# jqsl2012/RL_CTR_Prediction

Measured on NVIDIA B200. Metric: train samples/sec, higher is better.
Workload: dtype f32

## Files before the change

rl_ctr_prediction_b200/csrc/optim.cu:

```cuda
#include <cub/device/device_radix_sort.cuh>

#include <cstdlib>

#include "common.cuh"

namespace rlctr {

constexpr int LONG_RUN = 32;

struct TableView {
    float* data;
    int64_t n_rows;
    int rs, lin_col, emb_col, dim;
    int pitch;
    int used;
};
static inline TableView view_of(const rlctr_table* t) {
    int used = t->emb_col + t->dim;
    if (t->lin_col + 1 > used) used = t->lin_col + 1;
    if (used < 1) used = 1;
    return TableView{t->data, t->n_rows, t->row_stride, t->lin_col, t->emb_col, t->dim,
                     t->row_pitch > 0 ? t->row_pitch : t->row_stride, used};
}
struct AdamView {
    float* m;
    float* v;
    int32_t* stamp;
    int stamp_col;
    const float2* sched;
    const int32_t* step;
    AdamHyper h;
    const float* stage;
    int stage_pitch;
};
static inline int stage_pitch_of(const TableView& t) { return t.rs == 1 ? 4 : 3 * ((t.used + 3) & ~3); }
static inline AdamView view_of(const rlctr_adam* a, const TableView& t) {
    return AdamView{a->exp_avg, a->exp_avg_sq, a->stamp_col >= 0 ? nullptr : a->stamp, a->stamp_col >= 0 ? a->stamp_col : -1,
                    reinterpret_cast<const float2*>(a->sched), a->step,
                    adam_hyper(a->beta1, a->beta2, a->eps, a->weight_decay), a->stage, stage_pitch_of(t)};
}
__device__ __forceinline__ bool is_lazy(const AdamView& a) { return a.stamp != nullptr || a.stamp_col >= 0; }
__device__ __forceinline__ int load_stamp(const TableView& t, const AdamView& a, int64_t id) {
    return a.stamp_col >= 0 ? __float_as_int(t.data[id * t.pitch + a.stamp_col]) : a.stamp[id];
}
__device__ __forceinline__ void embed_stamp(float4& p, int col0, const AdamView& a, int value) {
    if (a.stamp_col >= 0 && (a.stamp_col & ~3) == col0) f4set(p, a.stamp_col & 3, __int_as_float(value));
}
struct GroupCols {
    int n;
    const float* dz[RLCTR_GROUP_MAX];
    const float* extra[RLCTR_GROUP_MAX];
    int emb_col[RLCTR_GROUP_MAX], dim[RLCTR_GROUP_MAX];
    const uint32_t* slot_of;
    int sums_pitch;
    signed char member[32];
    signed char role[32];
    int dz_used;
};
struct GradView {
    GroupCols grp;
    const float* staged;
    const float* dlogit;
    const float* sums;
    const float* extra;
    int fields;
    int flags;
    int world;
    uint32_t n_per_rank;
    const float* p_staged[RLCTR_MAX_WORLD];
    const float* p_dlogit[RLCTR_MAX_WORLD];
    const float* p_sums[RLCTR_MAX_WORLD];
    const float* p_extra[RLCTR_MAX_WORLD];
};
struct GradSrc {
    const float* staged;
    const float* dlogit;
    const float* sums;
    const float* extra;
    uint32_t slot;
};
__device__ __forceinline__ GradSrc grad_src(const GradView& g, uint32_t slot) {
    if (g.world <= 1) return GradSrc{g.staged, g.dlogit, g.sums, g.extra, slot};
    const uint32_t src = slot / g.n_per_rank;
    return GradSrc{g.p_staged[src], g.p_dlogit[src], g.p_sums[src], g.p_extra[src], slot - src * g.n_per_rank};
}
static inline GradView grad_view_of(const rlctr_rowgrad* grad) {
    GradView g{};
    g.staged = grad->staged; g.dlogit = grad->dlogit; g.sums = grad->sums; g.extra = grad->extra;
    g.fields = grad->fields; g.flags = grad->flags;
    g.world = grad->world; g.n_per_rank = grad->n_per_rank;
    if (grad->world > 1) {
        for (int r = 0; r < grad->world && r < RLCTR_MAX_WORLD; ++r) {
            g.p_staged[r] = grad->peer_staged[r]; g.p_dlogit[r] = grad->peer_dlogit[r];
            g.p_sums[r] = grad->peer_sums[r]; g.p_extra[r] = grad->peer_extra[r];
        }
        g.staged = grad->peer_staged[0]; g.dlogit = grad->peer_dlogit[0]; g.sums = grad->peer_sums[0]; g.extra = grad->peer_extra[0];
    }
    return g;
}

__global__ void __launch_bounds__(256)
sort_prep_kernel(const int64_t* __restrict__ ids, int64_t n, int64_t n_rows, uint32_t* __restrict__ keys,
                 uint32_t* __restrict__ vals) {
    for (int64_t i = (int64_t)blockIdx.x * blockDim.x + threadIdx.x; i < n; i += (int64_t)gridDim.x * blockDim.x) {
        const int64_t id = __ldg(ids + i);
        keys[i] = ((uint64_t)id < (uint64_t)n_rows) ? (uint32_t)id : (uint32_t)n_rows;
        vals[i] = (uint32_t)i;
    }
}

__global__ void __launch_bounds__(256)
sort_prep_sharded_kernel(const uint32_t* __restrict__ ids_all, int64_t n_all, int64_t n_rows_global, int shift, uint32_t mask,
                         uint32_t rank, uint32_t n_local, uint32_t* __restrict__ keys, uint32_t* __restrict__ vals) {
    for (int64_t i = (int64_t)blockIdx.x * blockDim.x + threadIdx.x; i < n_all; i += (int64_t)gridDim.x * blockDim.x) {
        const uint32_t id = __ldg(ids_all + i);
        const bool mine = (uint64_t)id < (uint64_t)n_rows_global && (id & mask) == rank;
        keys[i] = mine ? (id >> shift) : n_local;
        vals[i] = (uint32_t)i;
    }
}

struct GradRaw {
    float4 r;
    float4 S;
    float dz;
    float ex[4];
    bool fm, has_ex, any;
};
__device__ __forceinline__ GradRaw rowgrad_load(const GradView& g, uint32_t gslot, int col0, const TableView& t) {
    const GradSrc q = grad_src(g, gslot);
    const uint32_t slot = q.slot;
    GradRaw w;
    w.r = f4zero(); w.S = f4zero(); w.dz = 0.f; w.fm = false; w.has_ex = false; w.any = false;
#pragma unroll
    for (int k = 0; k < 4; ++k) w.ex[k] = 0.f;
    if (q.staged) w.r = ldg4(q.staged + (int64_t)slot * t.rs + col0);
    if (g.flags & RLCTR_STAGED_PARTNER) {
        w.dz = __ldg(q.dlogit + slot / (uint32_t)g.fields);
        return w;
    }
    if (q.dlogit || q.extra) {
        w.any = true;
        const uint32_t b = slot / (uint32_t)g.fields;
        const uint32_t f = slot - b * (uint32_t)g.fields;
        w.fm = q.sums && q.dlogit;
        if (w.fm && (g.flags & RLCTR_DZ_IN_SUMS)) w.dz = __ldg(q.sums + (int64_t)b * t.rs + (t.rs - 1));
        else if (q.dlogit) w.dz = __ldg(q.dlogit + b);
        if (w.fm) w.S = ldg4(q.sums + (int64_t)b * t.rs + col0);
        if (q.extra) {
            w.has_ex = true;
            const float* ex = q.extra + ((int64_t)b * g.fields + f) * t.dim;
#pragma unroll
            for (int k = 0; k < 4; ++k) {
                const int col = col0 + k;
                if (col >= t.emb_col && col < t.emb_col + t.dim) w.ex[k] = __ldg(ex + col - t.emb_col);
            }
        }
    }
    return w;
}
__device__ __forceinline__ float4 rowgrad_combine(const GradView& g, const GradRaw& w, int col0, const float4& p, const TableView& t) {
    float4 r = w.r;
    if (g.flags & RLCTR_STAGED_PARTNER) return make_float4(w.dz * r.x, w.dz * r.y, w.dz * r.z, w.dz * r.w);
    if (w.any) {
#pragma unroll
        for (int k = 0; k < 4; ++k) {
            const int col = col0 + k;
            float add = 0.f;
            if (col == t.lin_col) {
                add = w.dz;
            } else if (col >= t.emb_col && col < t.emb_col + t.dim) {
                if (w.fm) add = __fmul_rn(w.dz, f4get(w.S, k) - f4get(p, k));
                if (w.has_ex) add = __fadd_rn(add, w.ex[k]);
            }
            f4set(r, k, __fadd_rn(f4get(r, k), add));
        }
    }
    return r;
}
struct GroupLane {
    int mem[4], role[4];
};
__device__ __forceinline__ GroupLane group_lane(const GradView& g, int col0) {
    GroupLane gl;
#pragma unroll
    for (int k = 0; k < 4; ++k) {
        const int col = col0 + k;
        gl.mem[k] = col < 32 ? (int)g.grp.member[col] : -1;
        gl.role[k] = col < 32 ? (int)g.grp.role[col] : 0;
    }
    return gl;
}
__device__ __forceinline__ float group_col_grad(int role, float dz, float S, float p, bool has_ex, float ex) {
    float add = 0.f;
    if (role == 1) {
        add = dz;
    } else if (role != 0) {
        if (role == 2) add = __fmul_rn(dz, S - p);
        if (has_ex) add = __fadd_rn(add, ex);
    }
    return __fadd_rn(0.f, add);
}
__device__ __forceinline__ float4 rowgrad_group(const GradView& g, const GroupLane& gl, uint32_t slot, int col0, const float4& p,
                                                const TableView& t) {
    const uint32_t erow = slot;
    if (g.grp.slot_of) slot = __ldg(g.grp.slot_of + slot);
    const uint32_t b = slot / (uint32_t)g.fields;
    const float* srow = g.sums + (int64_t)b * g.grp.sums_pitch;
    const float4 S = ldg4(srow + col0);
    float4 r = f4zero();
#pragma unroll
    for (int k = 0; k < 4; ++k) {
        const int m = gl.mem[k];
        if (m < 0) continue;
        const float* dzp = g.grp.dz[m];
        const bool want_dz = gl.role[k] == 1 || gl.role[k] == 2;
        const float dz = !want_dz ? 0.f : dzp ? __ldg(dzp + b) : __ldg(srow + g.grp.sums_pitch - RLCTR_GROUP_MAX + m);
        const float* ex = gl.role[k] >= 2 ? g.grp.extra[m] : nullptr;
        const float exv = ex ? __ldg(ex + (int64_t)erow * g.grp.dim[m] + (col0 + k - g.grp.emb_col[m])) : 0.f;
        f4set(r, k, group_col_grad(gl.role[k], dz, f4get(S, k), f4get(p, k), ex != nullptr, exv));
    }
    return r;
}
template <bool GROUP>
__device__ __forceinline__ float4 rowgrad_any(const GradView& g, const GroupLane& gl, uint32_t slot, int col0, const float4& p,
                                              const TableView& t) {
    if (GROUP) return rowgrad_group(g, gl, slot, col0, p, t);
    return rowgrad_combine(g, rowgrad_load(g, slot, col0, t), col0, p, t);
}
__device__ __forceinline__ float4 rowgrad_chunk(const GradView& g, uint32_t gslot, int col0, const float4& p,
                                                const TableView& t) {
    return rowgrad_combine(g, rowgrad_load(g, gslot, col0, t), col0, p, t);
}

__device__ __forceinline__ void adam_apply4(float4& p, float4& m, float4& v, const float4& g, float2 s,
                                            const AdamHyper& h) {
    const float ib = rcp_approx(s.y);
    adam_elem_fast(p.x, m.x, v.x, g.x, h, s.x, ib);
    adam_elem_fast(p.y, m.y, v.y, g.y, h, s.x, ib);
    adam_elem_fast(p.z, m.z, v.z, g.z, h, s.x, ib);
    adam_elem_fast(p.w, m.w, v.w, g.w, h, s.x, ib);
}

template <int APPLY>
__device__ __forceinline__ void finish_row(int64_t id, int col0, float4 p, const float4& acc, const TableView& t,
                                           const AdamView& a, float* dense_grad, int step, int stamp_in,
                                           const float4* m_pre = nullptr, const float4* v_pre = nullptr) {
    if (APPLY == 1) {
        st4(dense_grad + id * t.rs + col0, acc);
        return;
    }
    const int64_t off = id * t.pitch + col0;
    float4 m = m_pre ? *m_pre : ld4(a.m + off), v = v_pre ? *v_pre : ld4(a.v + off);
    if (is_lazy(a) && !a.stage && stamp_in < step - 1) adam_replay4(p, m, v, stamp_in, step - 1, a.sched, a.h);
    adam_apply4(p, m, v, acc, __ldg(&a.sched[step]), a.h);
    embed_stamp(p, col0, a, step);
    st4(t.data + off, p);
    st4(a.m + off, m);
    st4(a.v + off, v);
}
// ... 981 lines not shown
    float* m[RLCTR_DENSE_MAX];
    float* v[RLCTR_DENSE_MAX];
    int64_t n[RLCTR_DENSE_MAX];
    int first_block[RLCTR_DENSE_MAX + 1];
    int step_index[RLCTR_DENSE_MAX];
    int count;
};
__global__ void __launch_bounds__(256)
dense_adam_multi_kernel(const __grid_constant__ DenseGroup grp, const float2* __restrict__ sched, const int32_t* __restrict__ steps,
                        AdamHyper h) {
    int t = 0;
    while (t + 1 < grp.count && (int)blockIdx.x >= grp.first_block[t + 1]) ++t;
    const float2 sc = __ldg(&sched[__ldg(steps + grp.step_index[t]) + 1]);
    const int nb = grp.first_block[t + 1] - grp.first_block[t];
    float* __restrict__ p = grp.p[t];
    const float* __restrict__ g = grp.g[t];
    float* __restrict__ m = grp.m[t];
    float* __restrict__ v = grp.v[t];
    for (int64_t i = (int64_t)(blockIdx.x - grp.first_block[t]) * blockDim.x + threadIdx.x; i < grp.n[t]; i += (int64_t)nb * blockDim.x) {
        float pp = p[i], mm = m[i], vv = v[i];
        adam_elem(pp, mm, vv, g[i], h, sc.x, sc.y);
        p[i] = pp; m[i] = mm; v[i] = vv;
    }
}

static inline int grid_1d(int64_t threads, int cap_blocks) {
    int64_t blocks = (threads + 255) / 256;
    if (blocks < 1) blocks = 1;
    return (int)(blocks < cap_blocks ? blocks : cap_blocks);
}
static inline int key_bits(int64_t n_rows) {
    int b = 1;
    while (b < 32 && ((int64_t)1 << b) <= n_rows) ++b;
    return b;
}
struct RowsWs {
    int32_t* long_count;
    uint32_t* long_list;
};
static inline size_t rows_ws_bytes(int64_t n) { return 16 + sizeof(uint32_t) * (size_t)(n / LONG_RUN + 1); }

static inline unsigned capped_blocks(int64_t full, int world) {
    if (world <= 1) return (unsigned)full;
    int64_t cap = full / world + full / (4 * world) + 2 * RLCTR_SMS;
    return (unsigned)(cap < full ? cap : full);
}

static inline int rows_grid_env() {
    static int v = -1;
    if (v < 0) { const char* e = getenv("RLCTR_ROWS_GRID"); v = e ? atoi(e) : 1; }
    return v;
}

template <int APPLY>
static int launch_rows(const uint32_t* sorted_ids, const uint32_t* sorted_slots, int64_t n, const rlctr_rowgrad* grad,
                       const rlctr_table* table, const rlctr_adam* opt, float* dense_grad, void* ws, size_t ws_bytes,
                       cudaStream_t st) {
    if (!sorted_ids || !sorted_slots || !grad || !table || !table->data || n < 0) return RLCTR_EINVAL;
    if (APPLY == 0 && (!opt || !opt->exp_avg || !opt->exp_avg_sq || !opt->sched || !opt->step)) return RLCTR_EINVAL;
    if (APPLY == 0 && opt->stamp_col >= (table->row_pitch > 0 ? table->row_pitch : table->row_stride)) return RLCTR_EINVAL;
    if (APPLY == 0 && opt->stamp_col >= 0 && table->row_stride > 32) return RLCTR_EUNSUPPORTED;
    if (APPLY == 1 && !dense_grad) return RLCTR_EINVAL;
    if ((grad->dlogit || grad->extra) && grad->fields <= 0) return RLCTR_EINVAL;
    if (n == 0) return RLCTR_OK;
    TableView t = view_of(table);
    AdamView a = APPLY == 0 ? view_of(opt, t) : AdamView{};
    if (grad->world > RLCTR_MAX_WORLD || (grad->world > 1 && grad->n_per_rank == 0)) return RLCTR_EINVAL;
    GradView g = grad_view_of(grad);
    if ((g.flags & RLCTR_STAGED_PARTNER) && (!g.staged || !g.dlogit || g.fields <= 0)) return RLCTR_EINVAL;
    if ((g.flags & RLCTR_DZ_IN_SUMS) && (t.rs <= t.used || !g.sums)) return RLCTR_EINVAL;
    if (t.rs == 1) {
        if (grad->extra || grad->sums) return RLCTR_EUNSUPPORTED;
        rows_scalar_kernel<APPLY><<<capped_blocks((n + 255) / 256, grad->world), 256, 0, st>>>(sorted_ids, sorted_slots, n, g, t, a,
                                                                                              dense_grad);
        RLCTR_LAUNCH_CHECK();
        return RLCTR_OK;
    }
    if (t.rs % 4 != 0 || t.rs > 128 * WCH) return RLCTR_EUNSUPPORTED;
    if (t.rs > 32) {
        rows_wide_kernel<APPLY><<<(unsigned)((n + 7) / 8), 256, 0, st>>>(sorted_ids, sorted_slots, n, g, t, a, dense_grad);
        RLCTR_LAUNCH_CHECK();
        return RLCTR_OK;
    }
    if (ws_bytes < rows_ws_bytes(n) || !ws) return RLCTR_EWORKSPACE;
    RowsWs w{reinterpret_cast<int32_t*>(ws), reinterpret_cast<uint32_t*>(reinterpret_cast<char*>(ws) + 16)};
    RLCTR_CUDA(cudaMemsetAsync(w.long_count, 0, sizeof(int32_t), st));
    const int lpr = rlctr_lanes_per_row(t.rs);
    unsigned blocks = capped_blocks((n * lpr + 255) / 256, grad->world);
    if (rows_grid_env() > 0 && blocks > (unsigned)(RLCTR_SMS * 5 * rows_grid_env())) blocks = RLCTR_SMS * 5 * rows_grid_env();
#define LAUNCH_ROWS(L)                                                                                              \
    rows_short_kernel<L, APPLY><<<blocks, 256, 0, st>>>(sorted_ids, sorted_slots, n, g, t, a, dense_grad,           \
                                                        w.long_count, w.long_list);                                \
    rows_long_kernel<L, APPLY><<<RLCTR_SMS, 256, 0, st>>>(sorted_ids, sorted_slots, n, g, t, a, dense_grad,         \
                                                          w.long_count, w.long_list)
    if (APPLY == 0 && a.stage && a.stamp == nullptr && lpr <= 4) {
        static int r_env = -1;
        if (r_env < 0) { const char* e = getenv("RLCTR_ROWS_R"); r_env = e ? atoi(e) : 0; }
        if (r_env == 0 && lpr == 4) {
            const int ch = (t.used + 3) >> 2;
            const int64_t tiles = capped_blocks((n + tile::TT - 1) / tile::TT, grad->world);
            const unsigned tb = (unsigned)(tiles < RLCTR_SMS * 3 ? tiles : RLCTR_SMS * 3);
#define LAUNCH_TILE(C)                                                                                                \
            { const size_t sm = 2 * sizeof(tile::Buf<C>);                                                             \
              RLCTR_CUDA(cudaFuncSetAttribute(rows_staged_tile_kernel<C>, cudaFuncAttributeMaxDynamicSharedMemorySize, (int)sm)); \
              rows_staged_tile_kernel<C><<<tb, 256, sm, st>>>(sorted_ids, sorted_slots, n, g, t, a, w.long_count, w.long_list); }
            switch (ch) {
                case 1: LAUNCH_TILE(1); break;
                case 2: LAUNCH_TILE(2); break;
                case 3: LAUNCH_TILE(3); break;
                default: LAUNCH_TILE(4); break;
            }
#undef LAUNCH_TILE
            RLCTR_LAUNCH_CHECK();
            rows_long_kernel<4, 0><<<RLCTR_SMS, 256, 0, st>>>(sorted_ids, sorted_slots, n, g, t, a, dense_grad, w.long_count, w.long_list);
            RLCTR_LAUNCH_CHECK();
            return RLCTR_OK;
        }
        const int R = r_env == 2 ? 2 : 4;
        const int64_t per_block = (256 / lpr) * R;
        int64_t want = (n + per_block - 1) / per_block;
        want = capped_blocks(want, grad->world);
        const int64_t cap = (int64_t)RLCTR_SMS * (R > 2 ? 2 : 3) * 4;
        const unsigned sblocks = (unsigned)(want < cap ? want : cap);
#define LAUNCH_STAGED(L)                                                                                              \
        if (R == 2) rows_staged_kernel<L, 2><<<sblocks, 256, 0, st>>>(sorted_ids, sorted_slots, n, g, t, a, w.long_count, w.long_list); \
        else rows_staged_kernel<L, 4><<<sblocks, 256, 0, st>>>(sorted_ids, sorted_slots, n, g, t, a, w.long_count, w.long_list);       \
        rows_long_kernel<L, 0><<<RLCTR_SMS, 256, 0, st>>>(sorted_ids, sorted_slots, n, g, t, a, dense_grad, w.long_count, w.long_list)
        switch (lpr) {
            case 1: LAUNCH_STAGED(1); break;
            case 2: LAUNCH_STAGED(2); break;
            default: LAUNCH_STAGED(4); break;
        }
#undef LAUNCH_STAGED
        RLCTR_COUNT_LAUNCH(1);
        RLCTR_LAUNCH_CHECK();
        return RLCTR_OK;
    }
    switch (lpr) {
        case 1: LAUNCH_ROWS(1); break;
        case 2: LAUNCH_ROWS(2); break;
        case 4: LAUNCH_ROWS(4); break;
        default: LAUNCH_ROWS(8); break;
    }
#undef LAUNCH_ROWS
    RLCTR_COUNT_LAUNCH(1);
    RLCTR_LAUNCH_CHECK();
    return RLCTR_OK;
}

}

using namespace rlctr;

extern "C" size_t rlctr_sort_ws_bytes(int64_t n, int64_t n_rows) {
    if (n <= 0) return 16;
    size_t temp = 0;
    cub::DeviceRadixSort::SortPairs(nullptr, temp, (const uint32_t*)nullptr, (uint32_t*)nullptr,
                                    (const uint32_t*)nullptr, (uint32_t*)nullptr, n, 0, key_bits(n_rows));
    size_t arr = ((size_t)n * sizeof(uint32_t) + 255) & ~(size_t)255;
    return 2 * arr + temp + 256;
}

extern "C" int rlctr_sort_ids(const int64_t* ids, int64_t n, int64_t n_rows, uint32_t* sorted_ids,
                              uint32_t* sorted_slots, void* ws, size_t ws_bytes, rlctr_stream_t stream) {
    if (!ids || !sorted_ids || !sorted_slots || !ws || n < 0 || n_rows <= 0) return RLCTR_EINVAL;
    if (n >= ((int64_t)1 << 32) || n_rows >= ((int64_t)1 << 32) - 1) return RLCTR_EUNSUPPORTED;
    if (n == 0) return RLCTR_OK;
    cudaStream_t st = (cudaStream_t)stream;
    size_t arr = ((size_t)n * sizeof(uint32_t) + 255) & ~(size_t)255;
    if (ws_bytes < 2 * arr + 256) return RLCTR_EWORKSPACE;
    uint32_t* keys = reinterpret_cast<uint32_t*>(ws);
    uint32_t* vals = reinterpret_cast<uint32_t*>(reinterpret_cast<char*>(ws) + arr);
    void* temp = reinterpret_cast<char*>(ws) + 2 * arr;
    size_t temp_bytes = ws_bytes - 2 * arr;
    sort_prep_kernel<<<grid_1d(n, RLCTR_SMS * 8), 256, 0, st>>>(ids, n, n_rows, keys, vals);
    RLCTR_LAUNCH_CHECK();
    cudaError_t e = cub::DeviceRadixSort::SortPairs(temp, temp_bytes, keys, sorted_ids, vals, sorted_slots, n, 0,
                                                    key_bits(n_rows), st);
    if (e != cudaSuccess) return (int)e;
    RLCTR_COUNT_LAUNCH(2 + (key_bits(n_rows) + 7) / 8);
    return RLCTR_OK;
}

extern "C" int rlctr_sort_ids_sharded(const uint32_t* ids_all, int64_t n_all, int32_t world, int32_t rank, int64_t n_rows_global,
                                      uint32_t* sorted_rows, uint32_t* sorted_slots, void* ws, size_t ws_bytes,
                                      rlctr_stream_t stream) {
    if (!ids_all || !sorted_rows || !sorted_slots || !ws || n_all < 0 || n_rows_global <= 0) return RLCTR_EINVAL;
    if (world != 1 && world != 2 && world != 4 && world != 8) return RLCTR_EUNSUPPORTED;
    if (rank < 0 || rank >= world) return RLCTR_EINVAL;
    if (n_all >= ((int64_t)1 << 32) || n_rows_global >= ((int64_t)1 << 32) - 1) return RLCTR_EUNSUPPORTED;
    if (n_all == 0) return RLCTR_OK;
    cudaStream_t st = (cudaStream_t)stream;
    int shift = 0;
    while ((1 << shift) < world) ++shift;
    const int64_t n_local = (n_rows_global - rank + world - 1) / world;
    size_t arr = ((size_t)n_all * sizeof(uint32_t) + 255) & ~(size_t)255;
    if (ws_bytes < 2 * arr + 256) return RLCTR_EWORKSPACE;
    uint32_t* keys = reinterpret_cast<uint32_t*>(ws);
    uint32_t* vals = reinterpret_cast<uint32_t*>(reinterpret_cast<char*>(ws) + arr);
    void* temp = reinterpret_cast<char*>(ws) + 2 * arr;
    size_t temp_bytes = ws_bytes - 2 * arr;
    sort_prep_sharded_kernel<<<grid_1d(n_all, RLCTR_SMS * 8), 256, 0, st>>>(ids_all, n_all, n_rows_global, shift, (uint32_t)(world - 1),
                                                                             (uint32_t)rank, (uint32_t)n_local, keys, vals);
    RLCTR_LAUNCH_CHECK();
    cudaError_t e = cub::DeviceRadixSort::SortPairs(temp, temp_bytes, keys, sorted_rows, vals, sorted_slots, n_all, 0,
                                                    key_bits(n_local), st);
    if (e != cudaSuccess) return (int)e;
    RLCTR_COUNT_LAUNCH(2 + (key_bits(n_local) + 7) / 8);
    return RLCTR_OK;
}

extern "C" size_t rlctr_rows_ws_bytes(int64_t n) { return rows_ws_bytes(n < 0 ? 0 : n); }

extern "C" int rlctr_rows_adam(const uint32_t* sorted_ids, const uint32_t* sorted_slots, int64_t n,
                               const rlctr_rowgrad* grad, const rlctr_table* table, const rlctr_adam* opt, void* ws,
                               size_t ws_bytes, rlctr_stream_t stream) {
    return launch_rows<0>(sorted_ids, sorted_slots, n, grad, table, opt, nullptr, ws, ws_bytes, (cudaStream_t)stream);
}

extern "C" int rlctr_group_rows_adam(const uint32_t* sorted_ids, const uint32_t* sorted_slots, int64_t n, const rlctr_table* table,
                                     const rlctr_adam* opt, const rlctr_member* members, int32_t n_members, const float* sums,
                                     int32_t sums_pitch, int32_t fields, int32_t world, const uint32_t* slot_of, void* ws,
                                     size_t ws_bytes, rlctr_stream_t stream) {
    if (!sorted_ids || !sorted_slots || !table || !table->data || !opt || !opt->exp_avg || !opt->exp_avg_sq || !opt->sched ||
        !opt->step || !members || !sums || n < 0 || fields <= 0)
        return RLCTR_EINVAL;
    if (n_members < 1 || n_members > RLCTR_GROUP_MAX) return RLCTR_EINVAL;
    if (table->world > 1 || opt->stage) return RLCTR_EUNSUPPORTED;
    if (n == 0) return RLCTR_OK;
    cudaStream_t st = (cudaStream_t)stream;
    TableView t = view_of(table);
    AdamView a = view_of(opt, t);
    if (t.rs % 4 != 0 || t.rs <= 8 || t.rs > 32) return RLCTR_EUNSUPPORTED;
    if (opt->stamp_col >= t.pitch) return RLCTR_EINVAL;
    if (!rlctr_aligned16(sums)) return RLCTR_EALIGN;
    if (sums_pitch == 0) sums_pitch = t.rs;
    if (sums_pitch < t.rs || sums_pitch % 4 != 0 || world < 0 || world > RLCTR_MAX_WORLD) return RLCTR_EINVAL;
    GradView g{};
    g.sums = sums; g.fields = fields; g.world = 0;
    g.grp.n = n_members;
    g.grp.sums_pitch = sums_pitch;
    g.grp.slot_of = slot_of;
    for (int col = 0; col < 32; ++col) { g.grp.member[col] = -1; g.grp.role[col] = 0; }
    for (int m = 0; m < n_members; ++m) {
        const rlctr_member& mm = members[m];
        if (mm.dim < 0 || mm.emb_col < 0 || mm.emb_col + mm.dim > t.rs || mm.lin_col >= t.rs) return RLCTR_EINVAL;
        const bool uses_dz = mm.lin_col >= 0 || ((mm.flags & RLCTR_FM_TERM) && mm.dim > 0);
        if (uses_dz && !mm.dlogit && sums_pitch - RLCTR_GROUP_MAX < t.rs) return RLCTR_EINVAL;
        if (uses_dz) g.grp.dz_used |= 1 << m;
        g.grp.dz[m] = mm.dlogit; g.grp.extra[m] = mm.extra; g.grp.emb_col[m] = mm.emb_col; g.grp.dim[m] = mm.dim;
        if (mm.lin_col >= 0) {
            if (g.grp.member[mm.lin_col] >= 0) return RLCTR_EINVAL;
            g.grp.member[mm.lin_col] = (signed char)m; g.grp.role[mm.lin_col] = 1;
        }
        for (int d = 0; d < mm.dim; ++d) {
            const int col = mm.emb_col + d;
            if (g.grp.member[col] >= 0) return RLCTR_EINVAL;
            g.grp.member[col] = (signed char)m; g.grp.role[col] = (mm.flags & RLCTR_FM_TERM) ? 2 : 3;
        }
    }
    if (opt->stamp_col >= 0 && opt->stamp_col < 32 && g.grp.member[opt->stamp_col] >= 0) return RLCTR_EINVAL;
    if (ws_bytes < rows_ws_bytes(n) || !ws) return RLCTR_EWORKSPACE;
    RowsWs w{reinterpret_cast<int32_t*>(ws), reinterpret_cast<uint32_t*>(reinterpret_cast<char*>(ws) + 16)};
    RLCTR_CUDA(cudaMemsetAsync(w.long_count, 0, sizeof(int32_t), st));
    const int lpr = rlctr_lanes_per_row(t.rs);
    const char* r2e = getenv("RLCTR_GROUP_ROWS2");
    const int rows2_env = r2e ? atoi(r2e) : 1;
    bool one_member_per_chunk = true;
    for (int ch = 0; ch < 8; ++ch) {
        int owner = -1;
        for (int q = 0; q < 4; ++q) {
            const int col = 4 * ch + q;
            if (g.grp.role[col] >= 2) {
                if (owner >= 0 && owner != g.grp.member[col]) one_member_per_chunk = false;
                owner = g.grp.member[col];
            }
        }
    }
    if (rows2_env && one_member_per_chunk && !opt->stamp && (t.used + 3) / 4 <= 8 && lpr == 8) {
        int64_t want = capped_blocks((2 * n + 255) / 256, world);
        const int64_t cap = (int64_t)RLCTR_SMS * 2 * (rows_grid_env() > 0 ? rows_grid_env() : 64);
        const unsigned b2 = (unsigned)(want < cap ? want : cap);
        if ((t.used + 3) / 4 <= 6) group_rows2_kernel<3><<<b2, 256, 0, st>>>(sorted_ids, sorted_slots, n, g, t, a, w.long_count, w.long_list);
        else group_rows2_kernel<4><<<b2, 256, 0, st>>>(sorted_ids, sorted_slots, n, g, t, a, w.long_count, w.long_list);
        rows_long_kernel<8, 0, true, 512><<<RLCTR_SMS, 512, 0, st>>>(sorted_ids, sorted_slots, n, g, t, a, nullptr, w.long_count, w.long_list);
        RLCTR_COUNT_LAUNCH(1);
        RLCTR_LAUNCH_CHECK();
        return RLCTR_OK;
    }
    unsigned blocks = capped_blocks((n * lpr + 255) / 256, world);
    if (rows_grid_env() > 0 && blocks > (unsigned)(RLCTR_SMS * 5 * rows_grid_env())) blocks = RLCTR_SMS * 5 * rows_grid_env();
    if (lpr == 4) {
        rows_short_kernel<4, 0, true><<<blocks, 256, 0, st>>>(sorted_ids, sorted_slots, n, g, t, a, nullptr, w.long_count, w.long_list);
        rows_long_kernel<4, 0, true><<<RLCTR_SMS, 256, 0, st>>>(sorted_ids, sorted_slots, n, g, t, a, nullptr, w.long_count, w.long_list);
    } else {
        rows_short_kernel<8, 0, true><<<blocks, 256, 0, st>>>(sorted_ids, sorted_slots, n, g, t, a, nullptr, w.long_count, w.long_list);
        rows_long_kernel<8, 0, true, 512><<<RLCTR_SMS, 512, 0, st>>>(sorted_ids, sorted_slots, n, g, t, a, nullptr, w.long_count, w.long_list);
    }
    RLCTR_COUNT_LAUNCH(1);
    RLCTR_LAUNCH_CHECK();
    return RLCTR_OK;
}

extern "C" int rlctr_rows_grad_dense(const uint32_t* sorted_ids, const uint32_t* sorted_slots, int64_t n,
                                     const rlctr_rowgrad* grad, const rlctr_table* table, float* dense_grad, void* ws,
                                     size_t ws_bytes, rlctr_stream_t stream) {
    return launch_rows<1>(sorted_ids, sorted_slots, n, grad, table, nullptr, dense_grad, ws, ws_bytes,
                          (cudaStream_t)stream);
}

extern "C" int64_t rlctr_lookup_stage_floats(const rlctr_table* table) {
    if (!table) return 0;
    return stage_pitch_of(view_of(table));
}

extern "C" int rlctr_rows_lookup(const uint32_t* sorted_ids, const uint32_t* sorted_slots, int64_t n, const rlctr_table* table,
                                 const rlctr_adam* opt, const rlctr_lookup* lookup, void* ws, size_t ws_bytes,
                                 rlctr_stream_t stream) {
    if (!sorted_ids || !sorted_slots || !table || !table->data || !opt || !opt->exp_avg || !opt->exp_avg_sq || !opt->sched ||
        !opt->step || !lookup || !lookup->stage || n < 0)
        return RLCTR_EINVAL;
    if (lookup->world > RLCTR_MAX_WORLD || (lookup->world > 1 && lookup->n_per_rank == 0)) return RLCTR_EINVAL;
// ... 167 lines not shown
```

Before: 48.52 million.

## Replace CUB device radix sort of embedding ids with custom bucket sort

Adds a two-level bucket sort for the id sort. A tiled histogram and scatter pass bins keys by their high bits into packed (low key bits, slot) words. Per-bucket block radix sorts then order each bucket, with a multi-pass fallback kernel for oversized buckets. The aim is fewer global radix passes and less memory traffic than cub::DeviceRadixSort. The cost is more kernels, atomics contention on skewed inputs, and a larger workspace. An env var can force the old CUB path.

Result: faster. 49.43 million, median of 6 (+1.9%).

```diff
diff --git a/rl_ctr_prediction_b200/csrc/optim.cu b/rl_ctr_prediction_b200/csrc/optim.cu
--- a/rl_ctr_prediction_b200/csrc/optim.cu
+++ b/rl_ctr_prediction_b200/csrc/optim.cu
@@ -1,3 +1,5 @@
+#include <cub/block/block_radix_sort.cuh>
+#include <cub/block/block_scan.cuh>
 #include <cub/device/device_radix_sort.cuh>
 
 #include <cstdlib>
@@ -99,13 +101,220 @@
     return g;
 }
 
+__device__ __forceinline__ uint32_t sort_key(int64_t id, int64_t n_rows) {
+    return ((uint64_t)id < (uint64_t)n_rows) ? (uint32_t)id : (uint32_t)n_rows;
+}
+
 __global__ void __launch_bounds__(256)
 sort_prep_kernel(const int64_t* __restrict__ ids, int64_t n, int64_t n_rows, uint32_t* __restrict__ keys,
                  uint32_t* __restrict__ vals) {
     for (int64_t i = (int64_t)blockIdx.x * blockDim.x + threadIdx.x; i < n; i += (int64_t)gridDim.x * blockDim.x) {
-        const int64_t id = __ldg(ids + i);
-        keys[i] = ((uint64_t)id < (uint64_t)n_rows) ? (uint32_t)id : (uint32_t)n_rows;
+        keys[i] = sort_key(__ldg(ids + i), n_rows);
         vals[i] = (uint32_t)i;
+    }
+}
+
+namespace bsort {
+constexpr int MAX_BUCKETS = 4096;
+constexpr int TILE_THREADS = 1024, TILE_ITEMS = 8, TILE = TILE_THREADS * TILE_ITEMS;
+constexpr int SMALL_THREADS = 128, SMALL_ITEMS = 4, SORT_THREADS = 256, BIG_ITEMS = 16;
+constexpr int SMALL = SMALL_THREADS * SMALL_ITEMS, BIG = SORT_THREADS * BIG_ITEMS;
+}
+
+__global__ void __launch_bounds__(bsort::TILE_THREADS)
+bucket_count_kernel(const int64_t* __restrict__ ids, int64_t n, int64_t n_rows, int low, int nb, uint32_t* __restrict__ totals,
+                    uint32_t* __restrict__ tile_off) {
+    __shared__ uint32_t hist[bsort::MAX_BUCKETS];
+    for (int b = threadIdx.x; b < nb; b += blockDim.x) hist[b] = 0;
+    __syncthreads();
+    const int64_t base = (int64_t)blockIdx.x * bsort::TILE + threadIdx.x;
+#pragma unroll
+    for (int j = 0; j < bsort::TILE_ITEMS; ++j) {
+        const int64_t i = base + j * bsort::TILE_THREADS;
+        if (i < n) atomicAdd(&hist[sort_key(__ldg(ids + i), n_rows) >> low], 1u);
+    }
+    __syncthreads();
+    for (int b = threadIdx.x; b < nb; b += blockDim.x)
+        if (hist[b]) tile_off[(int64_t)blockIdx.x * bsort::MAX_BUCKETS + b] = atomicAdd(&totals[b], hist[b]);
+}
+
+__global__ void __launch_bounds__(bsort::TILE_THREADS)
+bucket_scatter_kernel(const int64_t* __restrict__ ids, int64_t n, int64_t n_rows, int low, int slot_bits, int nb,
+                      const uint32_t* __restrict__ totals, const uint32_t* __restrict__ tile_off, uint32_t* __restrict__ bstart,
+                      uint32_t* __restrict__ comp) {
+    using Scan = cub::BlockScan<uint32_t, bsort::TILE_THREADS>;
+    constexpr int PER = bsort::MAX_BUCKETS / bsort::TILE_THREADS;
+    __shared__ typename Scan::TempStorage scan_tmp;
+    __shared__ uint32_t hist[bsort::MAX_BUCKETS];
+    uint32_t start[PER];
+#pragma unroll
+    for (int k = 0; k < PER; ++k) {
+        const int b = threadIdx.x * PER + k;
+        start[k] = b < nb ? totals[b] : 0u;
+        if (b < nb) hist[b] = 0;
+    }
+    Scan(scan_tmp).ExclusiveSum(start, start);
+    if (blockIdx.x == 0) {
+#pragma unroll
+        for (int k = 0; k < PER; ++k)
+            if (threadIdx.x * PER + k < nb) bstart[threadIdx.x * PER + k] = start[k];
+        if (threadIdx.x == 0) bstart[nb] = (uint32_t)n;
+    }
+    __syncthreads();
+    const uint32_t low_mask = (1u << low) - 1u;
+    const int64_t base = (int64_t)blockIdx.x * bsort::TILE + threadIdx.x;
+    uint32_t key[bsort::TILE_ITEMS], rank[bsort::TILE_ITEMS];
+#pragma unroll
+    for (int j = 0; j < bsort::TILE_ITEMS; ++j) {
+        const int64_t i = base + j * bsort::TILE_THREADS;
+        key[j] = i < n ? sort_key(__ldg(ids + i), n_rows) : 0u;
+        rank[j] = i < n ? atomicAdd(&hist[key[j] >> low], 1u) : 0u;
+    }
+    __syncthreads();
+#pragma unroll
+    for (int k = 0; k < PER; ++k) {
+        const int b = threadIdx.x * PER + k;
+        if (b < nb && hist[b]) hist[b] = start[k] + tile_off[(int64_t)blockIdx.x * bsort::MAX_BUCKETS + b];
+    }
+    __syncthreads();
+#pragma unroll
+    for (int j = 0; j < bsort::TILE_ITEMS; ++j) {
+        const int64_t i = base + j * bsort::TILE_THREADS;
+        if (i < n) comp[hist[key[j] >> low] + rank[j]] = ((key[j] & low_mask) << slot_bits) | (uint32_t)i;
+    }
+}
+
+__device__ __forceinline__ void bucket_emit(uint32_t* __restrict__ sorted_ids, uint32_t* __restrict__ sorted_slots, uint32_t b,
+                                            int low, int slot_bits, uint32_t pos, uint32_t c) {
+    sorted_ids[pos] = (uint32_t)((uint64_t)b << low) | (c >> slot_bits);
+    sorted_slots[pos] = c & ((1u << slot_bits) - 1u);
+}
+
+using BucketBigSort = cub::BlockRadixSort<uint32_t, bsort::SORT_THREADS, bsort::BIG_ITEMS>;
+using BucketScan = cub::BlockScan<uint32_t, bsort::SORT_THREADS>;
+__device__ __forceinline__ void bucket_sort_big(const uint32_t* __restrict__ bstart, uint32_t b, uint32_t* __restrict__ comp,
+                                                uint32_t* __restrict__ tmp, int low, int slot_bits, int bits,
+                                                uint32_t* __restrict__ sorted_ids, uint32_t* __restrict__ sorted_slots,
+                                                BucketBigSort::TempStorage& big_s, BucketScan::TempStorage& scan_s,
+                                                uint32_t* digit_base, uint32_t (*edge_key)[bsort::SORT_THREADS], int* first, int* last) {
+    using BigSort = BucketBigSort;
+    using Scan = BucketScan;
+    const int tid = threadIdx.x;
+    const uint32_t lo = bstart[b], m = bstart[b + 1] - lo;
+    if (m <= (uint32_t)bsort::BIG) {
+        uint32_t k[bsort::BIG_ITEMS];
+#pragma unroll
+        for (int j = 0; j < bsort::BIG_ITEMS; ++j) {
+            const uint32_t p = tid * bsort::BIG_ITEMS + j;
+            k[j] = p < m ? comp[lo + p] : 0xffffffffu;
+        }
+        BigSort(big_s).Sort(k, 0, bits);
+#pragma unroll
+        for (int j = 0; j < bsort::BIG_ITEMS; ++j) {
+            const uint32_t p = tid * bsort::BIG_ITEMS + j;
+            if (p < m) bucket_emit(sorted_ids, sorted_slots, b, low, slot_bits, lo + p, k[j]);
+        }
+        return;
+    }
+    uint32_t* src = comp + lo;
+    uint32_t* dst = tmp + lo;
+    for (int bit = 0; bit < bits; bit += 8) {
+        const int nbits = bits - bit < 8 ? bits - bit : 8;
+        const uint32_t dmask = (1u << nbits) - 1u;
+        const bool final_pass = bit + 8 >= bits;
+        digit_base[tid] = 0;
+        __syncthreads();
+        for (uint32_t i = tid; i < m; i += bsort::SORT_THREADS) atomicAdd(&digit_base[(src[i] >> bit) & dmask], 1u);
+        __syncthreads();
+        uint32_t c = digit_base[tid];
+        Scan(scan_s).ExclusiveSum(c, c);
+        digit_base[tid] = c;
+        for (uint32_t c0 = 0; c0 < m; c0 += bsort::BIG) {
+            const uint32_t cnt = m - c0 < (uint32_t)bsort::BIG ? m - c0 : (uint32_t)bsort::BIG;
+            uint32_t k[bsort::BIG_ITEMS];
+#pragma unroll
+            for (int j = 0; j < bsort::BIG_ITEMS; ++j) {
+                const uint32_t p = tid * bsort::BIG_ITEMS + j;
+                k[j] = p < cnt ? src[c0 + p] : 0xffffffffu;
+            }
+            __syncthreads();
+            first[tid] = -1;
+            BigSort(big_s).Sort(k, bit, bit + nbits);
+            edge_key[0][tid] = k[0];
+            edge_key[1][tid] = k[bsort::BIG_ITEMS - 1];
+            __syncthreads();
+#pragma unroll
+            for (int j = 0; j < bsort::BIG_ITEMS; ++j) {
+                const uint32_t p = tid * bsort::BIG_ITEMS + j;
+                if (p >= cnt) continue;
+                const uint32_t d = (k[j] >> bit) & dmask;
+                const uint32_t prev = j > 0 ? k[j - 1] : (tid > 0 ? edge_key[1][tid - 1] : 0u);
+                const uint32_t next = j + 1 < bsort::BIG_ITEMS ? k[j + 1] : (tid + 1 < bsort::SORT_THREADS ? edge_key[0][tid + 1] : 0u);
+                if (p == 0 || ((prev >> bit) & dmask) != d) first[d] = (int)p;
+                if (p + 1 == cnt || ((next >> bit) & dmask) != d) last[d] = (int)p;
+            }
+            __syncthreads();
+#pragma unroll
+            for (int j = 0; j < bsort::BIG_ITEMS; ++j) {
+                const uint32_t p = tid * bsort::BIG_ITEMS + j;
+                if (p >= cnt) continue;
+                const uint32_t d = (k[j] >> bit) & dmask;
+                const uint32_t pos = digit_base[d] + p - (uint32_t)first[d];
+                if (final_pass) bucket_emit(sorted_ids, sorted_slots, b, low, slot_bits, lo + pos, k[j]);
+                else dst[pos] = k[j];
+            }
+            __syncthreads();
+            if (first[tid] >= 0) digit_base[tid] += (uint32_t)(last[tid] - first[tid] + 1);
+        }
+        __syncthreads();
+        uint32_t* t = src; src = dst; dst = t;
+    }
+}
+
+__global__ void __launch_bounds__(bsort::SMALL_THREADS)
+bucket_sort_small_kernel(const uint32_t* __restrict__ bstart, const uint32_t* __restrict__ comp, int low, int slot_bits, int bits,
+                         uint32_t* __restrict__ big_count, uint32_t* __restrict__ big_list, uint32_t* __restrict__ sorted_ids,
+                         uint32_t* __restrict__ sorted_slots) {
+    using Sort = cub::BlockRadixSort<uint32_t, bsort::SMALL_THREADS, bsort::SMALL_ITEMS>;
+    __shared__ typename Sort::TempStorage tmp_s;
+    const uint32_t b = blockIdx.x;
+    const uint32_t lo = bstart[b], m = bstart[b + 1] - lo;
+    if (m == 0) return;
+    if (m > (uint32_t)bsort::SMALL) {
+        if (threadIdx.x == 0) big_list[atomicAdd(big_count, 1u)] = b;
+        return;
+    }
+    uint32_t k[bsort::SMALL_ITEMS];
+#pragma unroll
+    for (int j = 0; j < bsort::SMALL_ITEMS; ++j) {
+        const uint32_t p = threadIdx.x * bsort::SMALL_ITEMS + j;
+        k[j] = p < m ? comp[lo + p] : 0xffffffffu;
+    }
+    Sort(tmp_s).Sort(k, 0, bits);
+#pragma unroll
+    for (int j = 0; j < bsort::SMALL_ITEMS; ++j) {
+        const uint32_t p = threadIdx.x * bsort::SMALL_ITEMS + j;
+        if (p < m) bucket_emit(sorted_ids, sorted_slots, b, low, slot_bits, lo + p, k[j]);
+    }
+}
+
+__global__ void __launch_bounds__(bsort::SORT_THREADS)
+bucket_sort_big_kernel(const uint32_t* __restrict__ bstart, const uint32_t* __restrict__ big_count,
+                       const uint32_t* __restrict__ big_list, uint32_t* __restrict__ comp, uint32_t* __restrict__ tmp, int low,
+                       int slot_bits, int bits, uint32_t* __restrict__ sorted_ids, uint32_t* __restrict__ sorted_slots) {
+    using BigSort = cub::BlockRadixSort<uint32_t, bsort::SORT_THREADS, bsort::BIG_ITEMS>;
+    using Scan = cub::BlockScan<uint32_t, bsort::SORT_THREADS>;
+    __shared__ union {
+        typename BigSort::TempStorage big;
+        typename Scan::TempStorage scan;
+    } tmp_s;
+    __shared__ uint32_t digit_base[256], edge_key[2][bsort::SORT_THREADS];
+    __shared__ int first[256], last[256];
+    const uint32_t n_big = *big_count;
+    for (uint32_t q = blockIdx.x; q < n_big; q += gridDim.x) {
+        __syncthreads();
+        bucket_sort_big(bstart, big_list[q], comp, tmp, low, slot_bits, bits, sorted_ids, sorted_slots, tmp_s.big, tmp_s.scan,
+                        digit_base, edge_key, first, last);
     }
 }
 
@@ -1393,13 +1602,42 @@
 
 using namespace rlctr;
 
+struct BucketGeom {
+    int low, slot_bits, bits, nb;
+};
+static bool bucket_geom(int64_t n, int64_t n_rows, BucketGeom* g) {
+    if (n <= 0 || n >= ((int64_t)1 << 31)) return false;
+    const int kb = key_bits(n_rows);
+    int s = 0;
+    while (((int64_t)1 << s) < n) ++s;
+    int low = 0;
+    while (low < kb && (n << (low + 1)) <= 256 * (n_rows + 1)) ++low;
+    if (low > 31) low = 31;
+    if (low > 32 - s) low = 32 - s;
+    if (low < kb - 12) low = kb - 12;
+    if (low < 0) low = 0;
+    if (low + s > 32 || low > 31) return false;
+    *g = BucketGeom{low, s, low + s > 0 ? low + s : 1, 1 << (kb - low)};
+    return true;
+}
+static inline size_t bucket_ws_bytes(int64_t n) {
+    const size_t arr = ((size_t)n * sizeof(uint32_t) + 255) & ~(size_t)255;
+    const size_t tiles = (size_t)((n + bsort::TILE - 1) / bsort::TILE);
+    return 2 * arr + (3 + tiles) * sizeof(uint32_t) * bsort::MAX_BUCKETS + 512;
+}
+static inline bool sort_force_cub() {
+    const char* e = getenv("RLCTR_SORT_CUB");
+    return e && atoi(e) != 0;
+}
+
 extern "C" size_t rlctr_sort_ws_bytes(int64_t n, int64_t n_rows) {
     if (n <= 0) return 16;
     size_t temp = 0;
     cub::DeviceRadixSort::SortPairs(nullptr, temp, (const uint32_t*)nullptr, (uint32_t*)nullptr,
                                     (const uint32_t*)nullptr, (uint32_t*)nullptr, n, 0, key_bits(n_rows));
     size_t arr = ((size_t)n * sizeof(uint32_t) + 255) & ~(size_t)255;
-    return 2 * arr + temp + 256;
+    const size_t cub_bytes = 2 * arr + temp + 256;
+    return cub_bytes > bucket_ws_bytes(n) ? cub_bytes : bucket_ws_bytes(n);
 }
 
 extern "C" int rlctr_sort_ids(const int64_t* ids, int64_t n, int64_t n_rows, uint32_t* sorted_ids,
@@ -1409,6 +1647,31 @@
     if (n == 0) return RLCTR_OK;
     cudaStream_t st = (cudaStream_t)stream;
     size_t arr = ((size_t)n * sizeof(uint32_t) + 255) & ~(size_t)255;
+    BucketGeom g;
+    if (!sort_force_cub() && bucket_geom(n, n_rows, &g)) {
+        if (ws_bytes < bucket_ws_bytes(n)) return RLCTR_EWORKSPACE;
+        uint32_t* comp = reinterpret_cast<uint32_t*>(ws);
+        uint32_t* tmp = reinterpret_cast<uint32_t*>(reinterpret_cast<char*>(ws) + arr);
+        uint32_t* totals = reinterpret_cast<uint32_t*>(reinterpret_cast<char*>(ws) + 2 * arr);
+        uint32_t* big_count = totals + bsort::MAX_BUCKETS;
+        uint32_t* bstart = big_count + 32;
+        uint32_t* big_list = bstart + bsort::MAX_BUCKETS + 32;
+        uint32_t* tile_off = big_list + bsort::MAX_BUCKETS;
+        RLCTR_CUDA(cudaMemsetAsync(totals, 0, sizeof(uint32_t) * (bsort::MAX_BUCKETS + 32), st));
+        const unsigned tiles = (unsigned)((n + bsort::TILE - 1) / bsort::TILE);
+        bucket_count_kernel<<<tiles, bsort::TILE_THREADS, 0, st>>>(ids, n, n_rows, g.low, g.nb, totals, tile_off);
+        RLCTR_LAUNCH_CHECK();
+        bucket_scatter_kernel<<<tiles, bsort::TILE_THREADS, 0, st>>>(ids, n, n_rows, g.low, g.slot_bits, g.nb, totals, tile_off,
+                                                                      bstart, comp);
+        RLCTR_LAUNCH_CHECK();
+        bucket_sort_small_kernel<<<g.nb, bsort::SMALL_THREADS, 0, st>>>(bstart, comp, g.low, g.slot_bits, g.bits, big_count, big_list,
+                                                                         sorted_ids, sorted_slots);
+        RLCTR_LAUNCH_CHECK();
+        bucket_sort_big_kernel<<<RLCTR_SMS, bsort::SORT_THREADS, 0, st>>>(bstart, big_count, big_list, comp, tmp, g.low, g.slot_bits,
+                                                                           g.bits, sorted_ids, sorted_slots);
+        RLCTR_LAUNCH_CHECK();
+        return RLCTR_OK;
+    }
     if (ws_bytes < 2 * arr + 256) return RLCTR_EWORKSPACE;
     uint32_t* keys = reinterpret_cast<uint32_t*>(ws);
     uint32_t* vals = reinterpret_cast<uint32_t*>(reinterpret_cast<char*>(ws) + arr);
diff --git a/scratch/sort_ab.py b/scratch/sort_ab.py
--- /dev/null
+++ b/scratch/sort_ab.py
@@ -0,0 +1,112 @@
+import json
+import os
+import subprocess
+import sys
+
+import numpy as np
+import torch
+
+sys.path.insert(0, os.path.dirname(os.path.dirname(os.path.abspath(__file__))))
+from rl_ctr_prediction_b200 import _lib
+
+DEV = torch.device("cuda", 0)
+CALLS, BLOCK = 300, 10
+
+
+def c2_ids():
+    B, F, N = 65536, 15, 10_000_000
+    per = N // F
+    g = torch.Generator(device=DEV).manual_seed(1)
+    return (torch.randint(0, per, (B, F), generator=g, device=DEV) + torch.arange(F, device=DEV) * per).view(-1), N
+
+
+def zipf_ids():
+    N, n = 10_000_000, 65536 * 15
+    ids = np.minimum(np.random.default_rng(3).zipf(1.2, n) - 1, N - 1)
+    return torch.as_tensor(np.random.default_rng(4).permutation(N)[ids]).to(DEV), N
+
+
+def c1_ids():
+    card = [24, 40, 300_000, 35, 370, 5, 25_000, 50_000, 21, 14, 4, 4, 130, 5]
+    N, B = 1_000_000, 4096
+    card.append(N - sum(card))
+    rng = np.random.default_rng(6)
+    cols, base = [], 0
+    for c in card:
+        rank = np.minimum(np.floor(np.power(float(c), rng.random(B))).astype(np.int64) - 1, c - 1)
+        cols.append(base + np.maximum(rank, 0))
+        base += c
+    return torch.as_tensor(np.random.default_rng(7).permutation(N)[np.stack(cols, axis=1)]).view(-1).to(DEV), N
+
+
+def time_shape(lib, ids, n_rows):
+    n = ids.numel()
+    sid = torch.empty(n, dtype=torch.int32, device=DEV)
+    ss = torch.empty(n, dtype=torch.int32, device=DEV)
+    wsb = lib.rlctr_sort_ws_bytes(n, n_rows)
+    ws = torch.empty(wsb, dtype=torch.uint8, device=DEV)
+    st = _lib.stream()
+
+    def call():
+        assert lib.rlctr_sort_ids(_lib.ptr(ids), n, n_rows, _lib.ptr(sid), _lib.ptr(ss), _lib.ptr(ws), wsb, st) == 0
+
+    times = {"cub": [], "bucket": []}
+    outs = {}
+    for path in ("cub", "bucket"):
+        os.environ["RLCTR_SORT_CUB"] = "1" if path == "cub" else "0"
+        for _ in range(20):
+            call()
+        torch.cuda.synchronize()
+        outs[path] = (sid.clone(), ss.clone())
+    same = torch.equal(outs["cub"][0], outs["bucket"][0]) and torch.equal(outs["cub"][1], outs["bucket"][1])
+    ev = [(torch.cuda.Event(enable_timing=True), torch.cuda.Event(enable_timing=True)) for _ in range(BLOCK)]
+    for _ in range(CALLS // BLOCK):
+        for path in ("cub", "bucket"):
+            os.environ["RLCTR_SORT_CUB"] = "1" if path == "cub" else "0"
+            for e0, e1 in ev:
+                e0.record()
+                call()
+                e1.record()
+            torch.cuda.synchronize()
+            times[path] += [e0.elapsed_time(e1) * 1e3 for e0, e1 in ev]
+    os.environ.pop("RLCTR_SORT_CUB", None)
+    res = {"n": n, "n_rows": n_rows, "identical_outputs": same}
+    for path, t in times.items():
+        t = np.array(t)
+        res[path] = {"calls": len(t), "median_us": float(np.median(t)), "p10_us": float(np.percentile(t, 10)),
+                     "p90_us": float(np.percentile(t, 90)), "min_us": float(t.min())}
+    res["speedup_median"] = res["cub"]["median_us"] / res["bucket"]["median_us"]
+    from torch.profiler import ProfilerActivity, profile
+    for path in ("cub", "bucket"):
+        os.environ["RLCTR_SORT_CUB"] = "1" if path == "cub" else "0"
+        with profile(activities=[ProfilerActivity.CUDA]) as prof:
+            for _ in range(50):
+                call()
+            torch.cuda.synchronize()
+        ks = {}
+        for e in prof.events():
+            if e.device_type == torch.autograd.DeviceType.CUDA:
+                k = e.name.split("(")[0][:60]
+                ks.setdefault(k, []).append(e.time_range.end - e.time_range.start)
+        res[path]["kernels_us"] = {k: round(float(np.mean(v)), 2) for k, v in ks.items()}
+    os.environ.pop("RLCTR_SORT_CUB", None)
+    return res
+
+
+def main():
+    lib = _lib.load()
+    smi = subprocess.run(["nvidia-smi", "--query-gpu=name,power.limit,clocks.max.sm", "--format=csv,noheader"],
+                         capture_output=True, text=True).stdout.strip()
+    out = {"gpu": smi, "calls_per_path": CALLS, "alternation_block": BLOCK, "shapes": {}}
+    for name, fn in (("C2_uniform", c2_ids), ("C2_zipf1.2", zipf_ids), ("C1_campaign", c1_ids)):
+        ids, n_rows = fn()
+        out["shapes"][name] = time_shape(lib, ids.contiguous(), n_rows)
+        print(name, json.dumps(out["shapes"][name]), flush=True)
+    print("gpu:", smi)
+    if len(sys.argv) > 1:
+        with open(sys.argv[1], "w") as fh:
+            json.dump(out, fh, indent=1)
+
+
+if __name__ == "__main__":
+    main()
```
